# CobayaSampler/cobaya

Hardware: AMD Instinct MI355X
Metric: log-posterior evals/sec (whole node), 30-dim gaussian_mixture (higher is better)
Workload: dtype f64

## Files before the change

cobaya_amd/csrc/incremental_common.h:

```cpp
#pragma once
#include "det_math.h"
#include "kernels.h"

#ifndef MCMC_EXP_WAVES
#define MCMC_EXP_WAVES(family, tuned) (tuned)
#define MCMC_EXP_PIPE(tuned) (tuned)
#define MCMC_EXP_BLOCK_BEGIN() ((void)0)
#define MCMC_EXP_BLOCK_END() ((void)0)
#define MCMC_EXP_ROTATE_SHIFT(tuned) (tuned)
#define MCMC_EXP_ROTATE(on) (on)
#define MCMC_EXP_KEEP(tuned) (tuned)
#endif
#ifndef MCMC_EXP_FLOAT_BOUNDS
#define MCMC_EXP_FLOAT_BOUNDS(tuned) (tuned)
#endif
#ifndef MCMC_EXP_BOUNDS_LDS
#define MCMC_EXP_BOUNDS_LDS(tuned) (tuned)
#endif

namespace mcmc {
namespace {

template <int CTRL>
__device__ __forceinline__ double quad_perm(double v)
{
    int lo = __double2loint(v), hi = __double2hiint(v);
    lo = __builtin_amdgcn_mov_dpp(lo, CTRL, 0xf, 0xf, true);
    hi = __builtin_amdgcn_mov_dpp(hi, CTRL, 0xf, 0xf, true);
    return __hiloint2double(hi, lo);
}
__device__ __forceinline__ double quad_sum(double p)
{
    const double q = p + quad_perm<0xB1>(p);
    return q + quad_perm<0x4E>(q);
}

__device__ __forceinline__ unsigned quad_max_u32(unsigned v)
{
    unsigned o = (unsigned)__builtin_amdgcn_mov_dpp((int)v, 0xB1, 0xf, 0xf, true);
    v = v > o ? v : o;
    o = (unsigned)__builtin_amdgcn_mov_dpp((int)v, 0x4E, 0xf, 0xf, true);
    return v > o ? v : o;
}

__device__ __forceinline__ int hw_wave_slot()
{
    return (int)(__builtin_amdgcn_s_getreg(4 | (0 << 6) | (3 << 11)) & 15u);
}
template <int NW>
__device__ __forceinline__ void rotate_priority(int slot)
{
    if (!MCMC_EXP_ROTATE(true)) return;
    if (NW != 2 && NW != 4) return;
    const int turn = (int)(__builtin_amdgcn_s_memtime() >> MCMC_EXP_ROTATE_SHIFT(17));
    switch (NW == 4 ? ((slot + turn) & 3) : ((slot + turn) & 1)) {
    case 0: __builtin_amdgcn_s_setprio(0); break;
    case 1: __builtin_amdgcn_s_setprio(1); break;
    case 2: __builtin_amdgcn_s_setprio(2); break;
    default: __builtin_amdgcn_s_setprio(3); break;
    }
}

__device__ __forceinline__ unsigned long long quad_all_mask(unsigned long long m)
{
    m &= m >> 1;
    m &= m >> 2;
    m &= 0x1111111111111111ull;
    return m * 15ull;
}
__device__ __forceinline__ bool quad_all(unsigned long long m)
{
    return __builtin_amdgcn_inverse_ballot_w64(quad_all_mask(m));
}

typedef double __attribute__((ext_vector_type(2))) pair_t;
typedef const pair_t __attribute__((address_space(3))) * lds_pairs;
typedef const double __attribute__((address_space(3))) * lds_doubles;
typedef const double __attribute__((address_space(4))) * cdoubles;
__device__ __forceinline__ unsigned lds_offset(const void* p) { return (unsigned)(unsigned long long)p; }
__device__ __forceinline__ lds_pairs relaunder(const double2* p)
{
    unsigned off = lds_offset(p);
    asm volatile("" : "+v"(off));
    return (lds_pairs)(unsigned long long)off;
}
__device__ __forceinline__ lds_pairs relaunder_after(lds_pairs p, double anchor)
{
    unsigned off = (unsigned)(unsigned long long)p;
    asm volatile("" : "+v"(off) : "v"(anchor));
    return (lds_pairs)(unsigned long long)off;
}
__device__ __forceinline__ lds_doubles relaunder(const double* p)
{
    unsigned off = lds_offset(p);
    asm volatile("" : "+v"(off));
    return (lds_doubles)(unsigned long long)off;
}

template <bool hidden>
__device__ __forceinline__ void stage16_dma(void* lds_dst, const void* gsrc)
{
    if constexpr (hidden) {
        const unsigned dst = (unsigned)__builtin_amdgcn_readfirstlane((int)lds_offset(lds_dst));
        unsigned keep;
        asm volatile("s_mov_b32 %0, m0\n\ts_mov_b32 m0, %2\n\ts_nop 0\n\tglobal_load_lds_dwordx4 %1, off\n\ts_mov_b32 m0, %0"
                     : "=&s"(keep) : "v"(gsrc), "s"(dst) : "memory");
    } else {
        __builtin_amdgcn_global_load_lds((const __attribute__((address_space(1))) void*)gsrc,
                                         (__attribute__((address_space(3))) void*)lds_dst, 16, 0, 0);
    }
}
__device__ __forceinline__ void dma_wait() { asm volatile("s_waitcnt vmcnt(0)" ::: "memory"); }

#ifndef MCMC_STAGED_ROW
#define MCMC_STAGED_ROW 17
#endif
constexpr int kStagedRow = MCMC_STAGED_ROW;
constexpr int kStagedPairs = 4 * 8 * kStagedRow;
struct StagedVariates {
    unsigned base, off;
    __device__ __forceinline__ void init(const pair_t* sRE, int wave, int lane)
    {
        base = lds_offset(sRE + (wave * 8 * kStagedRow + (lane >> 2)));
        off = base;
    }
    __device__ __forceinline__ void fill(pair_t* sRE, int wave, int lane, int c, const PairRng& pr,
                                         unsigned long long S)
    {
        pair_t* const mine = sRE + ((wave * 8 + 2 * c) * kStagedRow + (lane >> 2));
        mine[0] = pair_t{pr.r[0], pr.Ea[0]};
        mine[kStagedRow] = pair_t{pr.r[1], pr.Ea[1]};
        off = base + (unsigned)(S & 7ull) * (16u * kStagedRow);
    }
    __device__ __forceinline__ void fetch(double& r, double& Ea) const
    {
        const pair_t re = *(lds_pairs)(unsigned long long)off;
        r = re.x;
        Ea = re.y;
    }
    __device__ __forceinline__ void next() { off += 16u * kStagedRow; }
};

constexpr int kMaxPeriodic = kIncMaxPeriodic;

__device__ __forceinline__ double pred_double(double x)
{
    const long long b = __double_as_longlong(x);
    if (x > 0.0) return __longlong_as_double(b - 1);
    if (x < 0.0) return __longlong_as_double(b + 1);
    return -4.9406564584124654e-324;
}


__host__ __device__ constexpr size_t inc_periodic_lds(int dq, int np)
{
    return sizeof(double) * (size_t)np * (64 + 4 * (size_t)dq);
}

__host__ __device__ constexpr int inc_chunk(int dq, bool with_w = false, bool per = false)
{
    if (per) {
        const int left = (dq <= 8 ? 40 : 80) * 1024 - 10752 - 64 * dq - 128 * dq -
                         (int)inc_periodic_lds(dq, kMaxPeriodic);
        int c = (left / (2 * (with_w ? 24 : 16)) / (4 * dq)) & ~3;
        return c < 4 ? 4 : (c > 64 ? 64 : c);
    }
    if (with_w) {
        int c = ((dq >= 9 ? 1364 : 600) / (4 * dq)) & ~3;
        return c < 8 ? 8 : (c > 64 ? 64 : c);
    }
    int c = ((dq >= 14 ? 2048 : 896) / (4 * dq)) & ~3;
    return c < 4 ? 4 : (c > 64 ? 64 : c);
}

}
}
```

cobaya_amd/csrc/incremental_duo.hip:

```cpp
#include <string>

#include "incremental_common.h"

#ifndef MCMC_DUO_DEPK
#define MCMC_DUO_DEPK(tuned) (tuned)
#endif
#ifndef MCMC_DUO_KEEPV
#define MCMC_DUO_KEEPV(tuned) (tuned)
#endif
#ifndef MCMC_DUO1_DMA_HIDDEN
#define MCMC_DUO1_DMA_HIDDEN 1
#endif
#ifndef MCMC_DUO1_LADDER
#define MCMC_DUO1_LADDER 4
#endif

namespace mcmc {
namespace {

__device__ __forceinline__ double pair_swap(double v) { return quad_perm<0xB1>(v); }
__device__ __forceinline__ double duo_sum(double p_even, double p_odd)
{
    const double s = p_even + p_odd;
    return s + pair_swap(s);
}
__device__ __forceinline__ unsigned pair_max_u32(unsigned v)
{
    const unsigned o = (unsigned)__builtin_amdgcn_mov_dpp((int)v, 0xB1, 0xf, 0xf, true);
    return v > o ? v : o;
}
__device__ __forceinline__ unsigned long long pair_all_mask(unsigned long long m)
{
    m &= m >> 1;
    m &= 0x5555555555555555ull;
    return m * 3ull;
}

constexpr int kDuoRow = 33;
constexpr int kDuoStagedPairs = 4 * 8 * kDuoRow;
struct DuoVariates {
    unsigned base, off;
    __device__ __forceinline__ void init(const pair_t* sRE, int wave, int lane)
    {
        base = lds_offset(sRE + (wave * 8 * kDuoRow + (lane >> 1)));
        off = base;
    }
    __device__ __forceinline__ void put(pair_t* sRE, int wave, int lane, int h, int q, const PairRng& p)
    {
        pair_t* const mine = sRE + ((wave * 8 + 4 * h + 2 * q) * kDuoRow + (lane >> 1));
        mine[0] = pair_t{p.r[0], p.Ea[0]};
        mine[kDuoRow] = pair_t{p.r[1], p.Ea[1]};
    }
    __device__ __forceinline__ void seek(unsigned long long S) { off = base + (unsigned)(S & 7ull) * (16u * kDuoRow); }
    __device__ __forceinline__ void fetch(double& r, double& Ea) const
    {
        const pair_t re = *(lds_pairs)(unsigned long long)off;
        r = re.x;
        Ea = re.y;
    }
    __device__ __forceinline__ void next() { off += 16u * kDuoRow; }
};

__host__ __device__ constexpr int duo_chunk_mix(int dq, int km)
{
    const int avail = 80 * 1024 - 16896 - 2560 - 2048 - (duo_x_in_lds(km, dq) ? dq * 4096 : 0);
    int c = ((avail / 16) / ((1 + km) * 4 * dq)) & ~3;
    return c < 4 ? 4 : (c > 64 ? 64 : c);
}
__host__ __device__ constexpr bool duo_keep_v(int dq, int km)
{
    return 2 * dq * (km + (duo_x_in_lds(km, dq) ? 0 : 1)) + 2 * dq <= 64;
}

template <int DQ, int KM, bool UNIT_T, bool BOX0>
__global__ void __launch_bounds__(256, 2) step_duo_mix_kernel(const IncStepArgs a)
{
    extern __shared__ __attribute__((aligned(16))) double smem[];
    constexpr int dpad = 4 * DQ;
    constexpr int NE = 2 * DQ;
    constexpr int COL = (1 + KM) * dpad;
    constexpr int C = duo_chunk_mix(DQ, KM);
    constexpr int CHUNK = C * COL;
    constexpr int DEPK = MCMC_DUO_DEPK(DQ / 2);
    constexpr bool XLDS = duo_x_in_lds(KM, DQ);
    constexpr bool KEEPV = MCMC_DUO_KEEPV(duo_keep_v(DQ, KM));
    const StepArgs& s = a.s;
    const int tid = threadIdx.x, h = tid & 1, wave = tid >> 6, lane = tid & 63;
    const int W = s.W, d = a.d;
    const int w = blockIdx.x * 128 + (tid >> 1);
    const int g = __builtin_amdgcn_readfirstlane(w / s.group_size);
    const int ncols = s.n_steps;
    const double* __restrict__ gVU = a.VU + (size_t)g * ncols * COL;
    auto stage = [&](int k) {
        const int first = k * C;
        if (first >= ncols) return;
        const int cols = ncols - first < C ? ncols - first : C;
        const int bytes = cols * COL * 8;
        const char* src = (const char*)(gVU + (size_t)first * COL);
        char* dst = (char*)(smem + (k & 1) * CHUNK);
        for (int kb = wave; kb * 1024 < bytes; kb += 4) {
            if (kb * 1024 + lane * 16 < bytes)
                stage16_dma<false>(dst + kb * 1024, src + kb * 1024 + lane * 16);
        }
    };
    stage(0);
    __shared__ double2 sLH[BOX0 ? 1 : 4 * DQ];
    __shared__ double2 sNA[BOX0 ? 1 : 4 * DQ];
    __shared__ double sNM[BOX0 ? 1 : 4 * DQ];
    if (!BOX0)
        for (int i = tid; i < dpad; i += 256) {
            sLH[i] = make_double2(a.prior[i], a.prior[dpad + i]);
            sNA[i] = make_double2(a.prior[2 * dpad + i], a.prior[3 * dpad + i]);
            sNM[i] = a.prior[4 * dpad + i];
        }
    double x[XLDS ? 1 : NE], y[KM][NE];
    typedef pair_t __attribute__((address_space(3))) * lds_pairs_rw;
    __shared__ pair_t sX[XLDS ? DQ * 256 : 1];
    const unsigned xoff0 = lds_offset(sX + tid);
#pragma unroll
    for (int kk = 0; kk < DQ; ++kk) {
        double xe[2];
#pragma unroll
        for (int j = 0; j < 2; ++j) {
            const int e = 2 * kk + j, i = 4 * kk + 2 * h + j;
            const bool in = i < d;
            xe[j] = in ? s.x[(size_t)i * W + w] : (BOX0 ? 0.5 * a.box_hi : 0.0);
            if (!XLDS) x[XLDS ? 0 : e] = xe[j];
#pragma unroll
            for (int k = 0; k < KM; ++k) y[k][e] = in ? a.y[((size_t)k * d + i) * W + w] : 0.0;
        }
        if (XLDS) sX[kk * 256 + tid] = pair_t{xe[0], xe[1]};
    }
    double cn[KM], wk[KM];
#pragma unroll
    for (int k = 0; k < KM; ++k) { cn[k] = s.cblock[a.cnorm_off + k]; wk[k] = s.cblock[a.weight_off + k]; }
    double lpost = s.logpost[w], lpri = s.logprior[w], llik = s.loglike[w];
    int wt = s.weight[w], prej = s.prior_rej[w], burn = s.burn_left[w];
    const long long nacc0 = s.n_accept[w];
    int nacc = 0;
    const uint32_t gid = s.walker0 + (uint32_t)w;
    const double mt10 = s.max_tries * 10.0;
    const int lim1 = s.max_tries < 2.0e9 ? (int)floor(s.max_tries) : 0x7fffffff;
    const int lim10 = mt10 < 2.0e9 ? (int)floor(mt10) : 0x7fffffff;
    __shared__ dpair_t short_log_lds[SHORT_LOG_TABLE_SIZE];
    const short_log_tab slog = short_log_load(short_log_lds);
    __shared__ double exp64_lds[64];
    const exp_tab etab = exp_tab_load(exp64_lds);
    dma_wait();
    __syncthreads();
    const unsigned long long half1 = 0xAAAAAAAAAAAAAAAAull;
    auto lse = [&](const double (&ak)[KM]) {
        double amax = ak[0];
#pragma unroll
        for (int k = 1; k < KM; ++k) amax = fmax(ak[k], amax);
        const double mine = sel(half1, ak[1], ak[0]);
        const double e_mine = dexp_tab(mine - amax, etab);
        double Ssum = fma(wk[0], quad_perm<0xA0>(e_mine), 0.0);
        Ssum = fma(wk[1], quad_perm<0xF5>(e_mine), Ssum);
        if (KM > 2) {
            const double mine2 = KM > 3 ? sel(half1, ak[3 < KM ? 3 : 0], ak[2 < KM ? 2 : 0]) : ak[2 < KM ? 2 : 0];
            const double e2 = dexp_tab(mine2 - amax, etab);
            Ssum = fma(wk[2 < KM ? 2 : 0], quad_perm<0xA0>(e2), Ssum);
            if (KM > 3) Ssum = fma(wk[3 < KM ? 3 : 0], quad_perm<0xF5>(e2), Ssum);
        }
        return dlog_tab(Ssum, slog) + amax;
    };
    double am[KM];
#pragma unroll
    for (int k = 0; k < KM; ++k) am[k] = a.amode[(size_t)k * W + w];
    if (a.anchor) {
#pragma unroll
        for (int k = 0; k < KM; ++k) {
            double pa0 = 0.0, pa1 = 0.0;
#pragma unroll
            for (int kk = 0; kk < DQ; ++kk) {
                pa0 = fma(y[k][2 * kk], y[k][2 * kk], pa0);
                pa1 = fma(y[k][2 * kk + 1], y[k][2 * kk + 1], pa1);
            }
            am[k] = -0.5 * (cn[k] + duo_sum(pa0, pa1));
        }
        llik = lse(am);
        lpost = lpri + llik;
    }
    const cdoubles gUU = (cdoubles)(unsigned long long)(a.UU + (size_t)g * ncols * KM);
    const unsigned bhi_word = (unsigned)__double2hiint(a.box_hi);
    const int hw_slot = hw_wave_slot();
    bool burning = lanes(burn > 0) != 0ull;
    unsigned long long cur_oct = ~0ull;
    __shared__ pair_t sRE[kDuoStagedPairs];
    DuoVariates sv;
    sv.init(sRE, wave, lane);

    for (int base = 0, kc = 0; base < ncols; base += C, ++kc) {
        const double* __restrict__ cur = smem + (kc & 1) * CHUNK;
        stage(kc + 1);
        const int cols = __builtin_amdgcn_readfirstlane(ncols - base < C ? ncols - base : C);
        unsigned coff = lds_offset(cur + 2 * h);
#pragma unroll 1
        for (int sl = 0; sl < cols; ++sl, coff += COL * 8) {
            const unsigned long long S = s.step0 + (unsigned long long)(base + sl);
            if ((S >> 3) != cur_oct) {
                cur_oct = S >> 3;
                rotate_priority<2>(hw_slot);
#pragma unroll 1
                for (int q = 0; q < 2; ++q) {
                    PairRng pr;
                    pr.run(s.key0, s.key1, gid, (cur_oct << 2) + (unsigned long long)(2 * h + q), slog);
                    sv.put(sRE, wave, lane, h, q, pr);
                }
                sv.seek(S);
            }
            double r, Ea;
            sv.fetch(r, Ea);
            sv.next();
            const lds_pairs col = (lds_pairs)(unsigned long long)coff;
            unsigned long long inb = ~0ull;
            double sc0 = 0.0, sc1 = 0.0;
            double dep;
            pair_t vk[KEEPV ? DQ : 1];
            unsigned xo = xoff0;
            if (XLDS) asm volatile("" : "+v"(xo));
            const lds_pairs xs = (lds_pairs)(unsigned long long)xo;
            auto xpair = [&](int kk) {
                if constexpr (XLDS) return xs[kk * 256];
                else return pair_t{x[2 * kk], x[2 * kk + 1]};
            };
            if constexpr (BOX0) {
                unsigned hmx = 0u;
#pragma unroll
                for (int kk = 0; kk < DQ; ++kk) {
                    const pair_t v = col[2 * kk];
                    const pair_t xp = xpair(kk);
                    if (KEEPV) vk[kk] = v;
                    if (kk == DEPK) dep = fma(r, v.x, xp.x);
                    const unsigned h0 = (unsigned)__double2hiint(fma(r, v.x, xp.x));
                    const unsigned h1 = (unsigned)__double2hiint(fma(r, v.y, xp.y));
                    hmx = hmx > h0 ? hmx : h0;
                    hmx = hmx > h1 ? hmx : h1;
                }
                inb = lanes(pair_max_u32(hmx) < bhi_word);
                if (inb != lanes(true)) {
                    unsigned xoff = coff;
                    asm volatile("" : "+v"(xoff));
                    const lds_pairs colx = (lds_pairs)(unsigned long long)xoff;
                    inb = ~0ull;
#pragma unroll
                    for (int kk = 0; kk < DQ; ++kk) {
                        const pair_t v = colx[2 * kk];
                        const pair_t xp = xpair(kk);
                        const double t0 = fma(r, v.x, xp.x), t1 = fma(r, v.y, xp.y);
                        inb &= lanes(t0 <= a.box_hi) & lanes(t0 >= 0.0);
                        inb &= lanes(t1 <= a.box_hi) & lanes(t1 >= 0.0);
                    }
                }
            } else {
#pragma unroll
                for (int kk = 0; kk < DQ; ++kk) {
                    const pair_t v = col[2 * kk];
                    const pair_t xp = xpair(kk);
                    if (KEEPV) vk[kk] = v;
#pragma unroll
                    for (int j = 0; j < 2; ++j) {
                        const int i = 4 * kk + 2 * h + j;
                        const double t = fma(r, j ? v.y : v.x, j ? xp.y : xp.x);
                        if (kk == DEPK && j == 0) dep = t;
                        const double2 lh = sLH[i];
                        inb &= lanes(t <= lh.y) & lanes(t >= lh.x);
                        if (a.has_norm) {
                            const double2 li = sNA[i];
                            const double qq = (t - li.x) * li.y;
                            if (j) sc1 = sc1 + fma(-0.5 * qq, qq, sNM[i]);
                            else sc0 = sc0 + fma(-0.5 * qq, qq, sNM[i]);
                        }
                    }
                }
            }
            double ak[KM];
#pragma unroll
            for (int k = 0; k < KM; ++k) {
                unsigned uoff = coff + (unsigned)((1 + k) * dpad * 8);
                asm volatile("" : "+v"(uoff) : "v"(dep));
                const lds_pairs uk = (lds_pairs)(unsigned long long)uoff;
                double pc0 = 0.0, pc1 = 0.0;
#pragma unroll
                for (int kk = 0; kk < DQ; ++kk) {
                    const pair_t u = uk[2 * kk];
                    pc0 = fma(y[k][2 * kk], u.x, pc0);
                    pc1 = fma(y[k][2 * kk + 1], u.y, pc1);
                    if (kk == DEPK) dep = pc0;
                }
                const double yu = duo_sum(pc0, pc1);
                const double uu = gUU[(size_t)(base + sl) * KM + k];
                ak[k] = fma(-0.5 * r, fma(r, uu, yu + yu), am[k]);
            }
            const unsigned long long inside_m = pair_all_mask(inb);
            const double lp = s.uniform_logp + ((!BOX0 && a.has_norm) ? duo_sum(sc0, sc1) : 0.0);
            const double ll = lse(ak);
            const double lt = lp + ll;
            const double delta = UNIT_T ? (lpost - lt) : (lpost - lt) / s.temperature;
            const unsigned long long acc_m = inside_m & (lanes(lt > lpost) | lanes(Ea > delta));
            const bool accept = __builtin_amdgcn_inverse_ballot_w64(acc_m);
            int lim = lim1;
            if (burning) {
                lim = burn > 0 ? lim10 : lim1;
                burn -= (accept & (burn > 0)) ? 1 : 0;
                burning = lanes(burn > 0) != 0ull;
            }
            const double ra = sel(acc_m, r, 0.0);
            if constexpr (XLDS) {
                unsigned xw = xoff0, poff = coff;
                asm volatile("" : "+v"(xw), "+v"(poff) : "v"(ra));
                const lds_pairs_rw px = (lds_pairs_rw)(unsigned long long)xw;
                const lds_pairs pv = (lds_pairs)(unsigned long long)poff;
#pragma unroll
                for (int kk = 0; kk < DQ; ++kk) {
                    pair_t xp = px[kk * 256];
                    pair_t v;
                    if constexpr (KEEPV) v = vk[kk];
                    else v = pv[2 * kk];
                    xp.x = fma(ra, v.x, xp.x);
                    xp.y = fma(ra, v.y, xp.y);
                    px[kk * 256] = xp;
                }
            } else if constexpr (KEEPV) {
#pragma unroll
                for (int kk = 0; kk < DQ; ++kk) {
                    x[2 * kk] = fma(ra, vk[kk].x, x[2 * kk]);
                    x[2 * kk + 1] = fma(ra, vk[kk].y, x[2 * kk + 1]);
                }
            } else {
                unsigned poff = coff;
                asm volatile("" : "+v"(poff) : "v"(ra));
                const lds_pairs pv = (lds_pairs)(unsigned long long)poff;
#pragma unroll
                for (int kk = 0; kk < DQ; ++kk) {
                    const pair_t v = pv[2 * kk];
                    x[2 * kk] = fma(ra, v.x, x[2 * kk]);
                    x[2 * kk + 1] = fma(ra, v.y, x[2 * kk + 1]);
                }
            }
#pragma unroll
            for (int k = 0; k < KM; ++k) {
                unsigned poff = coff + (unsigned)((1 + k) * dpad * 8);
                asm volatile("" : "+v"(poff) : "v"(k == 0 ? ((KEEPV || XLDS) ? ra : x[XLDS ? 0 : 2 * DEPK]) : y[k > 0 ? k - 1 : 0][2 * DEPK]));
                const lds_pairs pu = (lds_pairs)(unsigned long long)poff;
#pragma unroll
                for (int kk = 0; kk < DQ; ++kk) {
                    const pair_t u = pu[2 * kk];
                    y[k][2 * kk] = fma(ra, u.x, y[k][2 * kk]);
                    y[k][2 * kk + 1] = fma(ra, u.y, y[k][2 * kk + 1]);
                }
            }
#pragma unroll
            for (int k = 0; k < KM; ++k) am[k] = sel(acc_m, ak[k], am[k]);
            lpri = sel(acc_m, lp, lpri);
            llik = sel(acc_m, ll, llik);
            lpost = sel(acc_m, lt, lpost);
            prej = sel(acc_m, 0, prej + sel(inside_m, 0, 1));
            wt = sel(acc_m, 1, wt + 1);
            nacc += sel(acc_m, 1, 0);
            if (wt - prej > lim && h == 0) atomicCAS(s.stuck, 0, 1 + (int)gid);
        }
        dma_wait();
        __syncthreads();
    }
    int we = w, he = h;
    unsigned xe_off = xoff0;
    asm volatile("" : "+v"(we), "+v"(he), "+v"(xe_off));
    const lds_pairs xend = (lds_pairs)(unsigned long long)xe_off;
#pragma unroll
    for (int e = 0; e < NE; ++e) {
        const int i = 4 * (e >> 1) + 2 * he + (e & 1);
        if (i < d) {
            double xv;
            if constexpr (XLDS) { const pair_t xp = xend[(e >> 1) * 256]; xv = (e & 1) ? xp.y : xp.x; }
            else xv = x[XLDS ? 0 : e];
            s.x[(size_t)i * W + we] = xv;
#pragma unroll
            for (int k = 0; k < KM; ++k) a.y[((size_t)k * d + i) * W + we] = y[k][e];
        }
    }
    if (h == 0) {
#pragma unroll
        for (int k = 0; k < KM; ++k) a.amode[(size_t)k * W + we] = am[k];
        s.logpost[we] = lpost; s.logprior[we] = lpri; s.loglike[we] = llik;
        s.weight[we] = wt; s.prior_rej[we] = prej; s.burn_left[we] = burn;
        s.n_accept[we] = nacc0 + nacc;
    }
    wave_add_accepts(s.accept_total, (h == 0) ? nacc : 0);
}

template <int DQ, int KM>
hipError_t launch_duo_mix(const IncStepArgs& a, hipStream_t st)
{
    constexpr int C = duo_chunk_mix(DQ, KM);
    const size_t lds = sizeof(double) * 2 * C * (1 + KM) * 4 * DQ;
    const bool unit_t = a.s.temperature == 1.0;
    typedef void (*kern_t)(const IncStepArgs);
    const bool box0 = a.box && a.box_lo == 0.0 && a.box_hi > 0.0 && a.box_hi < INFINITY;
    static const kern_t kerns[4] = {
        step_duo_mix_kernel<DQ, KM, false, false>, step_duo_mix_kernel<DQ, KM, true, false>,
        step_duo_mix_kernel<DQ, KM, false, true>, step_duo_mix_kernel<DQ, KM, true, true>};
    const std::string stem = "mcmc::step_duo_mix_kernel<" + std::to_string(DQ) + ", " + std::to_string(KM);
    static const std::string names[4] = {stem + ", false>", stem + ", true>", stem + ", false, box>",
                                         stem + ", true, box>"};
    const int v = (unit_t ? 1 : 0) + (box0 ? 2 : 0);
    if (lds > 40 * 1024) {
        hipError_t e = hipFuncSetAttribute((const void*)kerns[v],
                                           hipFuncAttributeMaxDynamicSharedMemorySize, (int)lds);
        if (e != hipSuccess) return e;
    }
    mcmc_hip_note_step_kernel(names[v].c_str());
    hipLaunchKernelGGL(kerns[v], dim3(a.s.W / 128), dim3(256), lds, st, a);
    return hipGetLastError();
}

template <int DQ>
hipError_t dispatch_duo_mix(const IncStepArgs& a, hipStream_t st)
{
    if constexpr (DQ > MCMC_DUO_DQ_HI) {
        return hipErrorInvalidValue;
    } else {
        if (a.dq == DQ) {
            if (!duo_serves(a.n_modes, DQ)) return hipErrorInvalidValue;
            if constexpr (duo_serves(4, DQ)) {
                if (a.n_modes == 4) return launch_duo_mix<DQ, 4>(a, st);
            }
            if constexpr (duo_serves(3, DQ)) {
                if (a.n_modes == 3) return launch_duo_mix<DQ, 3>(a, st);
            }
            return a.n_modes == 2 ? launch_duo_mix<DQ, 2>(a, st) : hipErrorInvalidValue;
        }
        return dispatch_duo_mix<DQ + 1>(a, st);
    }
}

#if MCMC_DUO_DQ_LO == 1
#ifndef MCMC_DUO1_SPLIT
#define MCMC_DUO1_SPLIT 1
#endif
template <bool SPLIT>
__host__ __device__ constexpr int duo1_off(int e) { return SPLIT ? 2 * e : 4 * (e >> 1) + (e & 1); }
template <bool SPLIT>
__device__ __forceinline__ int duo1_dim(int e, int h) { return duo1_off<SPLIT>(e) + (SPLIT ? h : 2 * h); }
template <bool SPLIT>
__device__ __forceinline__ double duo1_sum(double q0, double q1)
{
    if constexpr (SPLIT) {
        const double lo = q0 + pair_swap(q0), hi = q1 + pair_swap(q1);
        return lo + hi;
    } else {
        return duo_sum(q0, q1);
    }
}
__host__ __device__ constexpr int duo1_chunk(int dq)
{
    int c = ((80 * 1024 - 16896 - 2048) / (2 * 64 * dq)) & ~3;
    return c > 64 ? 64 : c;
}

template <int DQ, int NE, bool SPLIT, bool UNIT_T>
__global__ void __launch_bounds__(256, 2) step_inc_duo_kernel(const IncStepArgs a)
{
    extern __shared__ __attribute__((aligned(16))) double2 smem2[];
    constexpr int COLB = 4 * DQ, dpad = 4 * DQ;
    constexpr int C = duo1_chunk(DQ);
    constexpr int CHUNK = C * COLB;
    static_assert(SPLIT ? (NE == 2 * DQ || NE == 2 * DQ - 1) : NE == 2 * DQ, "dimensions per lane");
    const StepArgs& s = a.s;
    const int tid = threadIdx.x, h = tid & 1, wave = tid >> 6, lane = tid & 63;
    const int W = s.W, d = a.d;
    const int w = blockIdx.x * 128 + (tid >> 1);
    const int g = __builtin_amdgcn_readfirstlane(w / s.group_size);
    const int ncols = s.n_steps;
    const int set_cols = a.vu_cols > 0 ? a.vu_cols : ncols;
    const double2* __restrict__ gVU = (const double2*)a.VU + ((size_t)g * set_cols + (size_t)a.col0) * COLB;
    auto stage = [&](int k) {
        const int first = k * C;
        if (first >= ncols) return;
        const int cols = ncols - first < C ? ncols - first : C;
        const int bytes = cols * COLB * 16;
        const char* src = (const char*)(gVU + (size_t)first * COLB);
        char* dst = (char*)(smem2 + (k & 1) * CHUNK);
        for (int kb = wave; kb * 1024 < bytes; kb += 4) {
            if (kb * 1024 + lane * 16 < bytes)
                stage16_dma<MCMC_DUO1_DMA_HIDDEN != 0>(dst + kb * 1024, src + kb * 1024 + lane * 16);
        }
    };
    const bool refresh_y = (a.anchor & 2) != 0;
    if (!refresh_y) stage(0);
    const double blo = a.box_lo, bhi = a.box_hi;
    const unsigned bhi_word = (unsigned)__double2hiint(bhi);
    double x[NE], y[NE];
#pragma unroll
    for (int e = 0; e < NE; ++e) {
        const int i = duo1_dim<SPLIT>(e, h);
        const bool in = i < d;
        x[e] = in ? s.x[(size_t)i * W + w] : 0.5 * (blo + bhi);
        y[e] = in ? a.y[(size_t)i * W + w] : 0.0;
    }
    double lpost = s.logpost[w], lpri = s.logprior[w], llik = s.loglike[w];
    __shared__ pair_t sRE[kDuoStagedPairs];
    if (refresh_y) {
        constexpr int TW = 8, SD = (dpad + TW - 1) / TW * TW;
        static_assert(128 * SD <= 4 * CHUNK, "the chunk buffers hold the deviations of the workgroup's walkers");
        static_assert(sizeof(pair_t) * kDuoStagedPairs >= sizeof(double) * dpad * TW, "the tile fits sRE");
        double* const sdev = (double*)smem2 + (size_t)(tid >> 1) * SD;
        double* const tile = (double*)sRE;
        for (int i = h; i < SD; i += 2) sdev[i] = 0.0;
#pragma unroll
        for (int e = 0; e < NE; ++e) {
            const int i = duo1_dim<SPLIT>(e, h);
            if (i < d) sdev[i] = x[e] - a.mean[i];
            y[e] = 0.0;
        }
        for (int i0 = 0; i0 < d; i0 += TW) {
            __syncthreads();
            for (int e = tid; e < dpad * TW; e += 256) {
                const int j = e / TW, i = i0 + e % TW;
                tile[e] = (j < d && i < d) ? a.Lrow[(size_t)j * d + i] : 0.0;
            }
            __syncthreads();
            const lds_doubles pt = relaunder(tile + (SPLIT ? h : 2 * h) * TW), pd = relaunder(sdev + i0);
#pragma unroll
            for (int ii = 0; ii < TW; ++ii) {
                const double dv = pd[ii];
#pragma unroll
                for (int e = 0; e < NE; ++e) y[e] = fma(pt[duo1_off<SPLIT>(e) * TW + ii], dv, y[e]);
            }
        }
        __syncthreads();
        stage(0);
    }
    if (a.anchor) {
        double pa0 = 0.0, pa1 = 0.0;
#pragma unroll
        for (int e = 0; e < NE; ++e) {
            if (e & 1) pa1 = fma(y[e], y[e], pa1);
            else pa0 = fma(y[e], y[e], pa0);
        }
        llik = -0.5 * (s.cnorm0 + duo1_sum<SPLIT>(pa0, pa1));
        lpost = lpri + llik;
    }
    int wt = s.weight[w], prej = s.prior_rej[w], burn = s.burn_left[w];
    long long nacc0 = s.n_accept[w];
    int nacc = 0;
    const cdoubles gUU = (cdoubles)(unsigned long long)(a.UU + (size_t)g * set_cols + (size_t)a.col0);
    const uint32_t gid = s.walker0 + (uint32_t)w;
    const double mt10 = s.max_tries * 10.0;
    const int lim1 = s.max_tries < 2.0e9 ? (int)floor(s.max_tries) : 0x7fffffff;
    const int lim10 = mt10 < 2.0e9 ? (int)floor(mt10) : 0x7fffffff;
    __shared__ dpair_t short_log_lds[SHORT_LOG_TABLE_SIZE];
    const short_log_tab slog = short_log_load(short_log_lds);
    dma_wait();
    __syncthreads();
    if constexpr (MCMC_DUO1_DMA_HIDDEN != 0) {
        asm volatile("" : "+v"(lpost), "+v"(lpri), "+v"(llik), "+v"(wt), "+v"(prej), "+v"(burn), "+v"(nacc0));
#pragma unroll
        for (int e = 0; e < NE; ++e) asm volatile("" : "+v"(x[e]), "+v"(y[e]));
    }
    bool burning = lanes(burn > 0) != 0ull;
    unsigned long long cur_oct = ~0ull;
    DuoVariates sv;
    sv.init(sRE, wave, lane);
    const int hw_slot = hw_wave_slot();

    for (int base = 0, k = 0; base < ncols; base += C, ++k) {
        const double2* __restrict__ cur = smem2 + (k & 1) * CHUNK;
        stage(k + 1);
        const int cols = __builtin_amdgcn_readfirstlane(ncols - base < C ? ncols - base : C);
        unsigned coff = lds_offset(cur + (SPLIT ? h : 2 * h));
#pragma unroll 1
        for (int sl = 0; sl < cols; ++sl, coff += COLB * 16) {
            const unsigned long long S = s.step0 + (unsigned long long)(base + sl);
            if ((S >> 3) != cur_oct) {
                cur_oct = S >> 3;
                rotate_priority<2>(hw_slot);
#pragma unroll 1
                for (int q = 0; q < 2; ++q) {
                    PairRng pr;
                    pr.run_lazy(s.key0, s.key1, gid, (cur_oct << 2) + (unsigned long long)(2 * h + q), slog);
                    sv.put(sRE, wave, lane, h, q, pr);
                }
                sv.seek(S);
            }
            double r, Ea;
            sv.fetch(r, Ea);
            sv.next();
            pair_t pk[NE];
            const lds_pairs col = (lds_pairs)(unsigned long long)coff;
#pragma unroll
            for (int e = 0; e < NE; ++e) pk[e] = col[duo1_off<SPLIT>(e)];
            unsigned hmx = 0u;
            double pc0 = 0.0, pc1 = 0.0;
            {
                constexpr int G = MCMC_DUO1_LADDER;
                static_assert(G >= 1, "pairs per rung");
                __builtin_amdgcn_sched_barrier(0);
#pragma unroll
                for (int e0 = 0; e0 < NE; e0 += G) {
                    const int e1 = e0 + G < NE ? e0 + G : NE;
#pragma unroll
                    for (int q = 0; q < e1 - e0; ++q) {
                        const int e = q == 0 ? e1 - 1 : e0 + q - 1;
                        const unsigned hw = (unsigned)__double2hiint(fma(r, pk[e].x, x[e]));
                        hmx = hmx > hw ? hmx : hw;
                    }
#pragma unroll
                    for (int e = e0; e < e1; ++e) {
                        if (e & 1) pc1 = fma(y[e], pk[e].y, pc1);
                        else pc0 = fma(y[e], pk[e].y, pc0);
                    }
                    __builtin_amdgcn_sched_barrier(0);
                }
                asm volatile("" : "+v"(pc0), "+v"(pc1));
            }
            const double uu = gUU[base + sl];
            unsigned long long inside_m = lanes(pair_max_u32(hmx) < bhi_word);
            if (inside_m != lanes(true)) {
                unsigned long long inb = ~0ull;
#pragma unroll
                for (int e = 0; e < NE; ++e) {
                    const double t = fma(r, pk[e].x, x[e]);
                    inb &= lanes(t <= bhi) & lanes(t >= blo);
                }
                inside_m = pair_all_mask(inb);
            }
            const double yu = duo1_sum<SPLIT>(pc0, pc1);
            const double mhr = -0.5 * r;
            const double lp = s.uniform_logp;
            const double ll = fma(mhr, fma(r, uu, yu + yu), llik);
            const double lt = lp + ll;
            const double delta = UNIT_T ? (lpost - lt) : (lpost - lt) / s.temperature;
            const unsigned long long up_m = UNIT_T ? 0ull : lanes(lt > lpost);
            const unsigned long long acc_m =
                inside_m & (up_m | accept_lanes(Ea, delta, a.accept_slack, s.key0, s.key1, gid, S, slog));
            const bool accept = __builtin_amdgcn_inverse_ballot_w64(acc_m);
            llik = accept ? ll : llik;
            int lim = lim1;
            if (burning) {
                lim = burn > 0 ? lim10 : lim1;
                burn -= (accept & (burn > 0)) ? 1 : 0;
                burning = lanes(burn > 0) != 0ull;
            }
            const double ra = accept ? r : 0.0;
#pragma unroll
            for (int e = 0; e < NE; ++e) {
                x[e] = fma(ra, pk[e].x, x[e]);
                y[e] = fma(ra, pk[e].y, y[e]);
            }
            lpost = accept ? lt : lpost;
            {
                const bool inside = __builtin_amdgcn_inverse_ballot_w64(inside_m);
                prej = accept ? 0 : (prej + (inside ? 0 : 1));
                wt = accept ? 1 : wt + 1;
                nacc += accept ? 1 : 0;
            }
            if (wt - prej > lim && h == 0) atomicCAS(s.stuck, 0, 1 + (int)gid);
        }
        dma_wait();
        __syncthreads();
    }
    int we = w, he = h;
    asm volatile("" : "+v"(we), "+v"(he));
#pragma unroll
    for (int e = 0; e < NE; ++e) {
        const int i = duo1_dim<SPLIT>(e, he);
        if (i < d) {
            s.x[(size_t)i * W + we] = x[e];
            a.y[(size_t)i * W + we] = y[e];
        }
    }
    if (h == 0) {
        s.logpost[we] = lpost; s.logprior[we] = lpri; s.loglike[we] = llik;
        s.weight[we] = wt; s.prior_rej[we] = prej; s.burn_left[we] = burn;
        s.n_accept[we] = nacc0 + nacc;
    }
    wave_add_accepts(s.accept_total, (h == 0) ? nacc : 0);
}

__global__ void __launch_bounds__(256) accept_estimate_error_kernel(double* err, uint32_t* at)
{
    __shared__ dpair_t short_log_lds[SHORT_LOG_TABLE_SIZE];
    const short_log_tab slog = short_log_load(short_log_lds);
    __shared__ double serr[256];
    __shared__ uint32_t sat[256];
    __syncthreads();
    const unsigned long long n = 1ull << 28, stride = (unsigned long long)gridDim.x * 256ull;
    double worst = -1.0;
    uint32_t where = 0u;
    for (unsigned long long k = 1ull + blockIdx.x * 256ull + threadIdx.x; k < n; k += stride) {
        const uint32_t ka = (uint32_t)k;
        const double e = fabs((double)accept_estimate(ka) - neg_log_short(2u * ka + 1u, 29, slog));
        if (e > worst || e != e) { worst = e; where = ka; }
    }
    serr[threadIdx.x] = worst;
    sat[threadIdx.x] = where;
    __syncthreads();
    if (threadIdx.x == 0) {
        for (int i = 1; i < 256; ++i)
            if (serr[i] > worst || serr[i] != serr[i]) { worst = serr[i]; where = sat[i]; }
        err[blockIdx.x] = worst;
        at[blockIdx.x] = where;
    }
}

template <int DQ, int NE, bool SPLIT>
hipError_t launch_duo1(const IncStepArgs& a, hipStream_t st)
{
    constexpr int C = duo1_chunk(DQ);
    const size_t lds = sizeof(double2) * 2 * C * 4 * DQ;
    const bool unit_t = a.s.temperature == 1.0;
    typedef void (*kern_t)(const IncStepArgs);
    static const kern_t kerns[2] = {step_inc_duo_kernel<DQ, NE, SPLIT, false>,
                                    step_inc_duo_kernel<DQ, NE, SPLIT, true>};
    static const std::string names[2] = {"mcmc::step_inc_kernel<" + std::to_string(DQ) + ", 0, false, two lanes>",
                                         "mcmc::step_inc_kernel<" + std::to_string(DQ) + ", 0, true, two lanes>"};
    const int v = unit_t ? 1 : 0;
    if (lds > 40 * 1024) {
        hipError_t e = hipFuncSetAttribute((const void*)kerns[v],
                                           hipFuncAttributeMaxDynamicSharedMemorySize, (int)lds);
        if (e != hipSuccess) return e;
    }
    mcmc_hip_note_step_kernel(names[v].c_str());
    hipLaunchKernelGGL(kerns[v], dim3(a.s.W / 128), dim3(256), lds, st, a);
    return hipGetLastError();
}

template <int DQ>
hipError_t dispatch_duo1(const IncStepArgs& a, hipStream_t st)
{
    if constexpr (DQ > kDuo1MaxDq) {
        return hipErrorInvalidValue;
    } else {
        if (a.dq != DQ) return dispatch_duo1<DQ + 1>(a, st);
        constexpr bool SPLIT = MCMC_DUO1_SPLIT != 0;
        if constexpr (SPLIT) {
            if ((a.d + 1) / 2 == 2 * DQ - 1) return launch_duo1<DQ, 2 * DQ - 1, true>(a, st);
            return launch_duo1<DQ, 2 * DQ, true>(a, st);
        } else {
            return launch_duo1<DQ, 2 * DQ, false>(a, st);
        }
    }
}
#endif

}
}

#define MCMC_CAT2(a, b) a##b
#define MCMC_CAT(a, b) MCMC_CAT2(a, b)
extern "C" hipError_t MCMC_CAT(mcmc_hip_launch_inc_duo_, MCMC_DUO_DQ_LO)(const mcmc::IncStepArgs* a,
                                                                       hipStream_t st)
{
    if (a->dq < MCMC_DUO_DQ_LO || a->dq > MCMC_DUO_DQ_HI || a->n_drag > 0 || a->colflag || a->s.rows ||
        a->s.W % 128 != 0 || a->s.group_size % 128 != 0)
        return hipErrorInvalidValue;
    for (int q = 0; q < 4; ++q)
        if (a->periodic_mask4[q]) return hipErrorInvalidValue;
    if (a->n_modes < 2 || !a->amode || a->vu_cols > 0) return hipErrorInvalidValue;
    return mcmc::dispatch_duo_mix<MCMC_DUO_DQ_LO>(*a, st);
}

#if MCMC_DUO_DQ_LO == 1
extern "C" hipError_t mcmc_hip_launch_inc_duo1(const mcmc::IncStepArgs* a, hipStream_t st)
{
    if (a->dq < 1 || a->dq > mcmc::kDuo1MaxDq || a->n_modes != 1 || a->n_drag > 0 || a->colflag || a->s.rows ||
        a->s.W % 128 != 0 || a->s.group_size % 128 != 0 || a->has_norm || !a->box || a->box_lo != 0.0 || !a->UU)
        return hipErrorInvalidValue;
    for (int q = 0; q < 4; ++q)
        if (a->periodic_mask4[q]) return hipErrorInvalidValue;
    return mcmc::dispatch_duo1<1>(*a, st);
}

extern "C" hipError_t mcmc_hip_launch_accept_estimate_error(double* err, uint32_t* ka, int n_blocks, hipStream_t st)
{
    if (n_blocks < 1) return hipErrorInvalidValue;
    hipLaunchKernelGGL(mcmc::accept_estimate_error_kernel, dim3(n_blocks), dim3(256), 0, st, err, ka);
    return hipGetLastError();
}
#endif
```

Baseline: 91.46 billion.

## Stage |u|^2 per chunk into LDS via DMA and split step loop by octets

Each chunk's |u|^2 values are now loaded into a double-buffered LDS region with global_load_lds_dword DMA alongside the proposal columns, so the per-step global uu load becomes an LDS read. The step loop is restructured into an outer loop over variate octets and an inner loop inside each octet, moving the seek and the octet check out of the per-step path. The stuck-chain atomic is deferred to once per chunk using an accumulated mask, and the bounds fallback gains extra early-exit hints. The extra LDS use is guarded by a static_assert to keep two workgroups per CU, and the UU load now goes out through a hidden M0-based asm DMA.

```diff
diff --git a/cobaya_amd/csrc/incremental_common.h b/cobaya_amd/csrc/incremental_common.h
--- a/cobaya_amd/csrc/incremental_common.h
+++ b/cobaya_amd/csrc/incremental_common.h
@@ -110,6 +110,13 @@
                                          (__attribute__((address_space(3))) void*)lds_dst, 16, 0, 0);
     }
 }
+__device__ __forceinline__ void stage4_dma(void* lds_dst, const void* gsrc)
+{
+    const unsigned dst = (unsigned)__builtin_amdgcn_readfirstlane((int)lds_offset(lds_dst));
+    unsigned keep;
+    asm volatile("s_mov_b32 %0, m0\n\ts_mov_b32 m0, %2\n\ts_nop 0\n\tglobal_load_lds_dword %1, off\n\ts_mov_b32 m0, %0"
+                 : "=&s"(keep) : "v"(gsrc), "s"(dst) : "memory");
+}
 __device__ __forceinline__ void dma_wait() { asm volatile("s_waitcnt vmcnt(0)" ::: "memory"); }
 
 #ifndef MCMC_STAGED_ROW
diff --git a/cobaya_amd/csrc/incremental_duo.hip b/cobaya_amd/csrc/incremental_duo.hip
--- a/cobaya_amd/csrc/incremental_duo.hip
+++ b/cobaya_amd/csrc/incremental_duo.hip
@@ -10,6 +10,9 @@
 #endif
 #ifndef MCMC_DUO1_DMA_HIDDEN
 #define MCMC_DUO1_DMA_HIDDEN 1
+#endif
+#ifndef MCMC_DUO1_UU_LDS
+#define MCMC_DUO1_UU_LDS 1
 #endif
 #ifndef MCMC_DUO1_LADDER
 #define MCMC_DUO1_LADDER 4
@@ -458,6 +461,10 @@
     int c = ((80 * 1024 - 16896 - 2048) / (2 * 64 * dq)) & ~3;
     return c > 64 ? 64 : c;
 }
+__host__ __device__ constexpr size_t duo1_lds(int dq)
+{
+    return (size_t)2 * duo1_chunk(dq) * (64 * dq + (MCMC_DUO1_UU_LDS != 0 ? 8 : 0));
+}
 
 template <int DQ, int NE, bool SPLIT, bool UNIT_T>
 __global__ void __launch_bounds__(256, 2) step_inc_duo_kernel(const IncStepArgs a)
@@ -466,6 +473,10 @@
     constexpr int COLB = 4 * DQ, dpad = 4 * DQ;
     constexpr int C = duo1_chunk(DQ);
     constexpr int CHUNK = C * COLB;
+    constexpr bool UU_LDS = MCMC_DUO1_UU_LDS != 0;
+    static_assert(duo1_lds(DQ) + sizeof(pair_t) * kDuoStagedPairs + sizeof(dpair_t) * SHORT_LOG_TABLE_SIZE <= 80 * 1024,
+                  "two workgroups per CU");
+    static_assert(2 * C <= 256, "a chunk's |u|^2: at most one dword per lane of the workgroup");
     static_assert(SPLIT ? (NE == 2 * DQ || NE == 2 * DQ - 1) : NE == 2 * DQ, "dimensions per lane");
     const StepArgs& s = a.s;
     const int tid = threadIdx.x, h = tid & 1, wave = tid >> 6, lane = tid & 63;
@@ -475,6 +486,8 @@
     const int ncols = s.n_steps;
     const int set_cols = a.vu_cols > 0 ? a.vu_cols : ncols;
     const double2* __restrict__ gVU = (const double2*)a.VU + ((size_t)g * set_cols + (size_t)a.col0) * COLB;
+    const double* __restrict__ gUUc = a.UU + ((size_t)g * set_cols + (size_t)a.col0);
+    double* const sUU = (double*)(smem2 + 2 * CHUNK);
     auto stage = [&](int k) {
         const int first = k * C;
         if (first >= ncols) return;
@@ -485,6 +498,10 @@
         for (int kb = wave; kb * 1024 < bytes; kb += 4) {
             if (kb * 1024 + lane * 16 < bytes)
                 stage16_dma<MCMC_DUO1_DMA_HIDDEN != 0>(dst + kb * 1024, src + kb * 1024 + lane * 16);
+        }
+        if constexpr (UU_LDS) {
+            if (wave * 64 + lane < 2 * cols)
+                stage4_dma((char*)(sUU + (k & 1) * C) + wave * 256, (const char*)(gUUc + first) + (wave * 64 + lane) * 4);
         }
     };
     const bool refresh_y = (a.anchor & 2) != 0;
@@ -564,17 +581,19 @@
     DuoVariates sv;
     sv.init(sRE, wave, lane);
     const int hw_slot = hw_wave_slot();
+    unsigned long long stuck_m = 0ull;
 
     for (int base = 0, k = 0; base < ncols; base += C, ++k) {
         const double2* __restrict__ cur = smem2 + (k & 1) * CHUNK;
         stage(k + 1);
         const int cols = __builtin_amdgcn_readfirstlane(ncols - base < C ? ncols - base : C);
         unsigned coff = lds_offset(cur + (SPLIT ? h : 2 * h));
+        unsigned uoff = lds_offset(sUU + (k & 1) * C);
 #pragma unroll 1
-        for (int sl = 0; sl < cols; ++sl, coff += COLB * 16) {
-            const unsigned long long S = s.step0 + (unsigned long long)(base + sl);
-            if ((S >> 3) != cur_oct) {
-                cur_oct = S >> 3;
+        for (int sl0 = 0; sl0 < cols;) {
+            const unsigned long long S0 = s.step0 + (unsigned long long)(base + sl0);
+            if ((S0 >> 3) != cur_oct) {
+                cur_oct = S0 >> 3;
                 rotate_priority<2>(hw_slot);
 #pragma unroll 1
                 for (int q = 0; q < 2; ++q) {
@@ -582,81 +601,104 @@
                     pr.run_lazy(s.key0, s.key1, gid, (cur_oct << 2) + (unsigned long long)(2 * h + q), slog);
                     sv.put(sRE, wave, lane, h, q, pr);
                 }
-                sv.seek(S);
-            }
-            double r, Ea;
-            sv.fetch(r, Ea);
-            sv.next();
-            pair_t pk[NE];
-            const lds_pairs col = (lds_pairs)(unsigned long long)coff;
-#pragma unroll
-            for (int e = 0; e < NE; ++e) pk[e] = col[duo1_off<SPLIT>(e)];
-            unsigned hmx = 0u;
-            double pc0 = 0.0, pc1 = 0.0;
-            {
-                constexpr int G = MCMC_DUO1_LADDER;
-                static_assert(G >= 1, "pairs per rung");
-                __builtin_amdgcn_sched_barrier(0);
-#pragma unroll
-                for (int e0 = 0; e0 < NE; e0 += G) {
-                    const int e1 = e0 + G < NE ? e0 + G : NE;
-#pragma unroll
-                    for (int q = 0; q < e1 - e0; ++q) {
-                        const int e = q == 0 ? e1 - 1 : e0 + q - 1;
-                        const unsigned hw = (unsigned)__double2hiint(fma(r, pk[e].x, x[e]));
-                        hmx = hmx > hw ? hmx : hw;
+            }
+            sv.seek(S0);
+            const int left = cols - sl0, in_oct = 8 - (int)(S0 & 7ull);
+            const int n_oct = left < in_oct ? left : in_oct;
+            [[maybe_unused]] const cdoubles uu_oct = gUU + (base + sl0);
+#pragma unroll 1
+            for (int so = 0; so < n_oct; ++so, coff += COLB * 16) {
+                int so_here = so;
+                asm volatile("" : "+s"(so_here));
+                double uu;
+                if constexpr (UU_LDS) {
+                    uu = *(lds_doubles)(unsigned long long)uoff;
+                    uoff += 8u;
+                }
+                double r, Ea;
+                sv.fetch(r, Ea);
+                sv.next();
+                pair_t pk[NE];
+                const lds_pairs col = (lds_pairs)(unsigned long long)coff;
+#pragma unroll
+                for (int e = 0; e < NE; ++e) pk[e] = col[duo1_off<SPLIT>(e)];
+                unsigned hmx = 0u;
+                double pc0 = 0.0, pc1 = 0.0;
+                {
+                    constexpr int G = MCMC_DUO1_LADDER;
+                    static_assert(G >= 1, "pairs per rung");
+                    __builtin_amdgcn_sched_barrier(0);
+#pragma unroll
+                    for (int e0 = 0; e0 < NE; e0 += G) {
+                        const int e1 = e0 + G < NE ? e0 + G : NE;
+#pragma unroll
+                        for (int q = 0; q < e1 - e0; ++q) {
+                            const int e = q == 0 ? e1 - 1 : e0 + q - 1;
+                            const unsigned hw = (unsigned)__double2hiint(fma(r, pk[e].x, x[e]));
+                            hmx = hmx > hw ? hmx : hw;
+                        }
+#pragma unroll
+                        for (int e = e0; e < e1; ++e) {
+                            if (e & 1) pc1 = fma(y[e], pk[e].y, pc1);
+                            else pc0 = fma(y[e], pk[e].y, pc0);
+                        }
+                        __builtin_amdgcn_sched_barrier(0);
                     }
-#pragma unroll
-                    for (int e = e0; e < e1; ++e) {
-                        if (e & 1) pc1 = fma(y[e], pk[e].y, pc1);
-                        else pc0 = fma(y[e], pk[e].y, pc0);
+                    asm volatile("" : "+v"(pc0), "+v"(pc1));
+                }
+                if constexpr (!UU_LDS) uu = uu_oct[so_here];
+                const unsigned pmx = pair_max_u32(hmx);
+                unsigned long long inside_m = lanes(pmx < bhi_word);
+                if (__builtin_expect(inside_m != lanes(true), 0)) {
+                    if (__builtin_expect((lanes(pmx == bhi_word) | lanes(pmx == 0x80000000u)) != 0ull, 0)) {
+                        unsigned long long inb = ~0ull;
+#pragma unroll
+                        for (int e = 0; e < NE; ++e) {
+                            const double t = fma(r, pk[e].x, x[e]);
+                            inb &= lanes(t <= bhi) & lanes(t >= blo);
+                        }
+                        inside_m = pair_all_mask(inb);
                     }
-                    __builtin_amdgcn_sched_barrier(0);
-                }
-                asm volatile("" : "+v"(pc0), "+v"(pc1));
-            }
-            const double uu = gUU[base + sl];
-            unsigned long long inside_m = lanes(pair_max_u32(hmx) < bhi_word);
-            if (inside_m != lanes(true)) {
-                unsigned long long inb = ~0ull;
+                }
+                const double yu = duo1_sum<SPLIT>(pc0, pc1);
+                const double mhr = -0.5 * r;
+                const double lp = s.uniform_logp;
+                const double ll = fma(mhr, fma(r, uu, yu + yu), llik);
+                const double lt = lp + ll;
+                const double delta = UNIT_T ? (lpost - lt) : (lpost - lt) / s.temperature;
+                const unsigned long long up_m = UNIT_T ? 0ull : lanes(lt > lpost);
+                const unsigned long long acc_m =
+                    inside_m & (up_m | accept_lanes(Ea, delta, a.accept_slack, s.key0, s.key1, gid,
+                                                    S0 + (unsigned long long)so_here, slog));
+                const bool accept = __builtin_amdgcn_inverse_ballot_w64(acc_m);
+                llik = accept ? ll : llik;
+                {
+                    const bool inside = __builtin_amdgcn_inverse_ballot_w64(inside_m);
+                    prej = accept ? 0 : (prej + (inside ? 0 : 1));
+                    wt = accept ? 1 : wt + 1;
+                    nacc += accept ? 1 : 0;
+                }
+                unsigned long long over_m = lanes(wt - prej > lim1);
+                if (__builtin_expect(burning, 0)) {
+                    const int lim = burn > 0 ? lim10 : lim1;
+                    burn -= (accept & (burn > 0)) ? 1 : 0;
+                    burning = lanes(burn > 0) != 0ull;
+                    over_m = lanes(wt - prej > lim);
+                }
+                stuck_m |= over_m;
+                const double ra = accept ? r : 0.0;
 #pragma unroll
                 for (int e = 0; e < NE; ++e) {
-                    const double t = fma(r, pk[e].x, x[e]);
-                    inb &= lanes(t <= bhi) & lanes(t >= blo);
-                }
-                inside_m = pair_all_mask(inb);
-            }
-            const double yu = duo1_sum<SPLIT>(pc0, pc1);
-            const double mhr = -0.5 * r;
-            const double lp = s.uniform_logp;
-            const double ll = fma(mhr, fma(r, uu, yu + yu), llik);
-            const double lt = lp + ll;
-            const double delta = UNIT_T ? (lpost - lt) : (lpost - lt) / s.temperature;
-            const unsigned long long up_m = UNIT_T ? 0ull : lanes(lt > lpost);
-            const unsigned long long acc_m =
-                inside_m & (up_m | accept_lanes(Ea, delta, a.accept_slack, s.key0, s.key1, gid, S, slog));
-            const bool accept = __builtin_amdgcn_inverse_ballot_w64(acc_m);
-            llik = accept ? ll : llik;
-            int lim = lim1;
-            if (burning) {
-                lim = burn > 0 ? lim10 : lim1;
-                burn -= (accept & (burn > 0)) ? 1 : 0;
-                burning = lanes(burn > 0) != 0ull;
-            }
-            const double ra = accept ? r : 0.0;
-#pragma unroll
-            for (int e = 0; e < NE; ++e) {
-                x[e] = fma(ra, pk[e].x, x[e]);
-                y[e] = fma(ra, pk[e].y, y[e]);
-            }
-            lpost = accept ? lt : lpost;
-            {
-                const bool inside = __builtin_amdgcn_inverse_ballot_w64(inside_m);
-                prej = accept ? 0 : (prej + (inside ? 0 : 1));
-                wt = accept ? 1 : wt + 1;
-                nacc += accept ? 1 : 0;
-            }
-            if (wt - prej > lim && h == 0) atomicCAS(s.stuck, 0, 1 + (int)gid);
+                    x[e] = fma(ra, pk[e].x, x[e]);
+                    y[e] = fma(ra, pk[e].y, y[e]);
+                }
+                lpost = accept ? lt : lpost;
+            }
+            sl0 += n_oct;
+        }
+        if (__builtin_expect(stuck_m != 0ull, 0)) {
+            if (__builtin_amdgcn_inverse_ballot_w64(stuck_m) && h == 0) atomicCAS(s.stuck, 0, 1 + (int)gid);
+            stuck_m = 0ull;
         }
         dma_wait();
         __syncthreads();
@@ -709,7 +751,8 @@
 hipError_t launch_duo1(const IncStepArgs& a, hipStream_t st)
 {
     constexpr int C = duo1_chunk(DQ);
-    const size_t lds = sizeof(double2) * 2 * C * 4 * DQ;
+    const size_t lds = duo1_lds(DQ);
+    static_assert(duo1_lds(DQ) >= sizeof(double2) * 2 * C * 4 * DQ, "the pairs' buffers");
     const bool unit_t = a.s.temperature == 1.0;
     typedef void (*kern_t)(const IncStepArgs);
     static const kern_t kerns[2] = {step_inc_duo_kernel<DQ, NE, SPLIT, false>,
```

After: 98.38 billion, median of 6. 1.08x the previous value.
